# lutteropp/QuartetScores

Hardware: AMD Instinct MI355X
Metric: quartets counted/sec (higher is better)
Workload: dtype u32

## Files before the change

### quartetscores_amd/csrc/qs_count.hip

```cpp
#include "qs_common.hpp"
#include "qs_internal.hpp"
#include "qs_bitslice3.hpp"

#include <cstdio>
#include <cstdlib>
#include <type_traits>
#include <vector>

namespace qs {


constexpr int kPanelThreads = 256;
constexpr int kPanelPPT = 8;
constexpr int kPanelPB = kPanelThreads * kPanelPPT;

template <typename DT, bool PARTIAL>
__global__ __launch_bounds__(kPanelThreads) void build_panel_kernel(const uint32_t *__restrict__ leaf_off,
                                                                    const uint32_t *__restrict__ order, uint32_t slot0,
                                                                    const uint16_t *__restrict__ leaf_ids,
                                                                    const uint16_t *__restrict__ adj_depth,
                                                                    uint32_t n_trees, uint32_t n, uint32_t npairs,
                                                                    uint32_t levels, uint4 *__restrict__ P) {
    constexpr int TPC = 16 / (int)sizeof(DT);
    constexpr uint32_t FLAG = sizeof(DT) == 1 ? 0x20u : 0x2000u;
// ... 612 lines not shown
constexpr int c4_hi_words(int nwords) { return nwords <= 4 ? 0 : nwords == 5 ? 1 : nwords == 6 ? 2 : 4; }


template <int B> constexpr int bs4_waves() { return B <= 4 ? 5 : 4; }
template <int B, typename CT>
__global__ __launch_bounds__(kCountThreads) __attribute__((amdgpu_waves_per_eu(bs4_waves<B>(), bs4_waves<B>()))) void count_bitslice4_kernel(
    const uint4 *__restrict__ P, uint32_t npairs, uint32_t n_groups, uint32_t m_trees, uint32_t d_start, uint32_t d_hi,
    uint64_t rank_lo, uint32_t n_dblk, uint32_t n_slots, const uint32_t *__restrict__ dprefix, const uint32_t *__restrict__ cprefix,
    CT *__restrict__ table, uint32_t *__restrict__ overflow_flag, uint32_t overwrite, uint32_t xcd_remap, uint32_t *__restrict__ wire,
    const uint32_t *__restrict__ perm) {
    constexpr int NB = B + 1;
    constexpr int NWRAW = B < 4 ? 4 : B;
    constexpr int HR = c4_hi_words(NWRAW), HI = c4_hi_words(NB);
    __shared__ uint4 raw_lo[2][kC4Raw];
    __shared__ __align__(16) uint32_t raw_hi[2][HR ? kC4Raw * HR : 4];
    __shared__ uint4 img_lo[kWavesPerBlock][kWave];
    __shared__ __align__(16) uint32_t img_hi[kWavesPerBlock][HI ? kWave * HI : 4];

    const uint32_t lane = threadIdx.x & (kWave - 1);
    const uint32_t wave = __builtin_amdgcn_readfirstlane(threadIdx.x / kWave);
    uint32_t lb = blockIdx.x;
    if (xcd_remap & 1u) {
        const uint32_t nb = gridDim.x, q8 = nb / 8, r8 = nb % 8, xcd = lb % 8, y = lb / 8;
        lb = (xcd < r8 ? xcd * (q8 + 1) : r8 * (q8 + 1) + (xcd - r8) * q8) + y;
    }
    uint32_t tile = (uint32_t)__builtin_amdgcn_readfirstlane((int)perm[lb * kWavesPerBlock + wave]);
    const bool shadow = (tile & kShadowTile) != 0;
    tile &= ~kShadowTile;
    uint32_t dp_k, cp_c;
    const uint32_t k = wave_search_le(dprefix, 0, n_dblk, tile, lane, dp_k);
    const uint32_t local = tile - dp_k;
    const uint32_t d1 = d_hi - k * kDB;
    const uint32_t d0 = d1 > d_start + kDB ? d1 - kDB : d_start;
    const uint32_t c = wave_search_le(cprefix, 2, d1 - 1, local, lane, cp_c);
    const uint32_t tl = local - cp_c;
    uint32_t Bk = (uint32_t)(2.0f * sqrtf((float)tl + 1.0f));
    while ((Bk * Bk) / 4 > tl) --Bk;
    while (((Bk + 1) * (Bk + 1)) / 4 <= tl) ++Bk;
    const uint32_t jt = tl - (Bk * Bk) / 4;
    const uint32_t blk0 = 2 * jt, blk1 = 2 * jt + 1;
    const uint32_t ia = lane & (kTA - 1), ib = lane / kTA;
    const uint32_t a1 = blk0 * kTA + ia, a2 = blk1 * kTA + ia, b = Bk * kTB + ib;
    const bool v1 = !shadow && b < c, v2 = v1;
    const uint32_t pi1 = (uint32_t)binom2(b) + a1, pi2 = (uint32_t)binom2(b) + a2;
    const uint32_t jlo = c >= d0 ? c + 1 - d0 : 0u, jhi = d1 - d0;

    const uint32_t r_j = lane >> 3, r_col = lane & 7, dE = d0 + r_j;
    uint32_t shoff = kS3Inv;
    if (wave == 0) shoff = pi1 * 16u;
    else if (wave == 1) shoff = pi2 * 16u;
    else if (wave == 2) { const uint32_t bE = Bk * kTB + r_col; if (dE < d1 && bE < dE) shoff = ((uint32_t)binom2(dE) + bE) * 16u; }
    uint32_t pvoff = kS3Inv;
    if (lane < 16) { const uint32_t xa = (lane < 8 ? blk0 : blk1) * kTA + (lane & 7); if (xa < c) pvoff = ((uint32_t)binom2(c) + xa) * 16u; }
    else if (lane < 24) { const uint32_t dy = d0 + (lane - 16); if (dy < d1 && dy > c) pvoff = ((uint32_t)binom2(dy) + c) * 16u; }
    const uint32_t group_bytes = npairs * (uint32_t)(NWRAW * 4), hi_base = npairs * 16u;
    const uint32_t pv_slot = kC4Shared + wave * kC4Private;

    uint32_t x0[kDB], x1[kDB], y0[kDB], y1[kDB];
#pragma unroll
    for (int j = 0; j < kDB; ++j) x0[j] = x1[j] = y0[j] = y1[j] = 0;

    auto rsrc_of = [&](uint32_t g) {
        return __builtin_amdgcn_make_buffer_rsrc((void *)(reinterpret_cast<const char *>(P) + (size_t)g * group_bytes), 0, (int)group_bytes, 0x00020000);
    };
    auto put_raw = [&](int bufi, const Planes &sh, const Planes &pv) {
        if (wave < 3) c4_put<NWRAW>(raw_lo[bufi], raw_hi[bufi], wave * kWave + lane, sh);
        if (lane < kC4Private) c4_put<NWRAW>(raw_lo[bufi], raw_hi[bufi], pv_slot + lane, pv);
    };
    auto step = [&](uint32_t g_next, auto cur_tag, auto full_tag) {
        constexpr int CUR = decltype(cur_tag)::value;
        constexpr bool FULL = decltype(full_tag)::value;
        asm volatile("s_waitcnt lgkmcnt(0)\n\ts_barrier" ::: "memory");
        const Planes ab1 = c4_get<NWRAW>(raw_lo[CUR], raw_hi[CUR], lane);
        const Planes rowA1 = c4_get<NWRAW>(raw_lo[CUR], raw_hi[CUR], pv_slot + ia);
        const Planes ab2 = c4_get<NWRAW>(raw_lo[CUR], raw_hi[CUR], kWave + lane);
        const Planes rowA2 = c4_get<NWRAW>(raw_lo[CUR], raw_hi[CUR], pv_slot + 8 + ia);
        const Planes mbd = c4_get<NWRAW>(raw_lo[CUR], raw_hi[CUR], 2 * kWave + lane);
        const Planes mcd = c4_get<NWRAW>(raw_lo[CUR], raw_hi[CUR], pv_slot + 16 + r_j);
        const __amdgpu_buffer_rsrc_t r = rsrc_of(g_next);
        const Planes sh = buf_load_planes<NWRAW>(r, shoff, hi_base);
        const Planes pv = buf_load_planes<NWRAW>(r, pvoff, hi_base);
        c4_put<NB>(img_lo[wave], img_hi[wave], lane, sub_biased<B>(mbd, mcd));
        const Planes L1 = sub_biased<B>(ab1, rowA1);
        const Planes L2 = sub_biased<B>(ab2, rowA2);
#pragma unroll
        for (int j = 0; j < kDB; ++j) {
            if (FULL || ((uint32_t)j >= jlo && (uint32_t)j < jhi)) {
                const Planes Rb = c4_get<NB>(img_lo[wave], img_hi[wave], j * 8 + ib);
                uint32_t gt, lt, gt2, lt2;
                cmp_planes<NB>(L1, Rb, gt, lt);
                popc_acc(gt, x0[j]);
                popc_acc(lt, x1[j]);
                cmp_planes<NB>(L2, Rb, gt2, lt2);
                popc_acc(gt2, y0[j]);
                popc_acc(lt2, y1[j]);
            }
        }
        put_raw(CUR ^ 1, sh, pv);
    };
    auto run = [&](auto full_tag) {
        using Z_ = std::integral_constant<int, 0>; using O_ = std::integral_constant<int, 1>;
        {
            const __amdgpu_buffer_rsrc_t r = rsrc_of(0);
            put_raw(0, buf_load_planes<NWRAW>(r, shoff, hi_base), buf_load_planes<NWRAW>(r, pvoff, hi_base));
        }
        const uint32_t g_last = n_groups - 1;
        uint32_t g = 0;
        for (; g + 2 <= n_groups; g += 2) {
            step(g + 1, Z_{}, full_tag);
            step(min(g + 2, g_last), O_{}, full_tag);
        }
        if (g < n_groups) step(g_last, Z_{}, full_tag);
    };
    if (jlo == 0 && jhi == (uint32_t)kDB) run(std::true_type{}); else run(std::false_type{});

    uint64_t bd4 = binom4(d0), bd3 = binom3(d0), bd2 = binom2(d0);
    const uint64_t rcb = binom3(c) - rank_lo;
    if (wire) {
#pragma unroll
        for (int j = 0; j < kDB; ++j) {
            const uint32_t d = d0 + j;
            const uint64_t base = bd4 + rcb;
            bd4 += bd3; bd3 += bd2; bd2 += d;
            if (d < d1 && d > c && v1) {
                uint32_t w = x0[j] | (x1[j] << 16), w2 = y0[j] | (y1[j] << 16);
                if (!overwrite) { w += wire[base + pi1]; w2 += wire[base + pi2]; }
                wire[base + pi1] = w;
                wire[base + pi2] = w2;
            }
        }
        return;
    }
#pragma unroll
    for (int j = 0; j < kDB; ++j) {
        const uint32_t d = d0 + j;
        const uint64_t base = bd4 + rcb;
        bd4 += bd3; bd3 += bd2; bd2 += d;
        if (d < d1 && d > c && v1) {
            {
                const uint64_t idx = (base + pi1) * 3;
                uint32_t w0 = x0[j], w1 = x1[j], w2 = m_trees - x0[j] - x1[j];
                if (!overwrite) { const Tuple3<CT> t = load_tuple(table + idx); w0 += t.a; w1 += t.b; w2 += t.c; }
                if (sizeof(CT) == 2 && ((w0 | w1 | w2) > 0xFFFFu)) atomicOr(overflow_flag, 1u);
                store_tuple(table + idx, w0, w1, w2);
            }
            if (v2) {
                const uint64_t idx = (base + pi2) * 3;
                uint32_t w0 = y0[j], w1 = y1[j], w2 = m_trees - y0[j] - y1[j];
                if (!overwrite) { const Tuple3<CT> t = load_tuple(table + idx); w0 += t.a; w1 += t.b; w2 += t.c; }
                if (sizeof(CT) == 2 && ((w0 | w1 | w2) > 0xFFFFu)) atomicOr(overflow_flag, 1u);
                store_tuple(table + idx, w0, w1, w2);
            }
        }
    }
}


hipError_t launch_count_bitslice3(hipStream_t s, const CountGeometry &g_in, const void *panel, int depth_bits, int mode,
                                  uint32_t n_groups, uint32_t m_trees, void *table, int count_bits, uint32_t *overflow_flag,
                                  bool overwrite, uint32_t *wire) {
    if (g_in.total_tiles == 0 || n_groups == 0) return hipSuccess;
    const uint32_t npairs = (uint32_t)binom2(g_in.n);
    CountGeometry g = g_in;
    if (mode == MODE_BINARY_FULL && g.perm_coop && g.n_coop && depth_bits <= 7) {
        dim3 grid4(g.n_coop / kWavesPerBlock), block4(kCountThreads);
#define QS_BS4(BB, CT)                                                                                              \
    hipLaunchKernelGGL((count_bitslice4_kernel<BB, CT>), grid4, block4, 0, s, (const uint4 *)panel, npairs, n_groups, m_trees, \
                       g.d_lo, g.d_hi, g.rank_lo, g.n_dblk, g.n_coop, g.dprefix, g.cprefix, (CT *)table, overflow_flag,    \
                       overwrite ? 1u : 0u, 1u, wire, g.perm_coop)
#define QS_BS4_B(CT)                                                                                                \
    do {                                                                                                            \
        if (depth_bits <= 4) QS_BS4(4, CT);                                                                         \
        else if (depth_bits == 5) QS_BS4(5, CT);                                                                    \
        else if (depth_bits == 6) QS_BS4(6, CT);                                                                    \
        else QS_BS4(7, CT);                                                                                         \
    } while (0)
        if (count_bits == 32) QS_BS4_B(uint32_t); else QS_BS4_B(uint16_t);
#undef QS_BS4_B
#undef QS_BS4
        hipError_t e4 = hipGetLastError();
        if (e4 != hipSuccess) return e4;
        g.perm = g.perm_rest; g.total_tiles = g.n_rest;
        if (g.total_tiles == 0) return hipSuccess;
    }
    dim3 grid((g.total_tiles + kWavesPerBlock - 1) / kWavesPerBlock), block(kCountThreads);
#define QS_BS3(BB, MM, CT)                                                                                          \
    hipLaunchKernelGGL((count_bitslice3_kernel<BB, MM, CT>), grid, block, 0, s, (const uint4 *)panel, npairs, n_groups, \
                       m_trees, g.d_lo, g.d_hi, g.rank_lo, g.n_dblk, g.total_tiles, g.dprefix, g.cprefix,           \
                       (CT *)table, overflow_flag, overwrite ? 1u : 0u, g.n >= 200 ? (((kSyncModes >> (MM)) & 1u) ? 3u : 1u) : 0u , wire, g.perm)
#define QS_BS3_B(MM, CT)                                                                                            \
    do {                                                                                                            \
        switch (depth_bits <= 4 ? 4 : depth_bits) {                                                                 \
            case 4: QS_BS3(4, MM, CT); break;                                                                       \
            case 5: QS_BS3(5, MM, CT); break;                                                                       \
            case 6: QS_BS3(6, MM, CT); break;                                                                       \
            case 7: QS_BS3(7, MM, CT); break;                                                                       \
            case 8: QS_BS3(8, MM, CT); break;                                                                       \
            case 9: QS_BS3(9, MM, CT); break;                                                                       \
            default: QS_BS3(10, MM, CT); break;                                                                     \
        }                                                                                                           \
    } while (0)
#define QS_BS3_BP(CT) QS_BS3_B(MODE_PARTIAL, CT)
    if (depth_bits > kMaxDepthBits) return hipErrorInvalidValue;
    if (count_bits == 32) {
        if (mode == MODE_BINARY_FULL) QS_BS3_B(MODE_BINARY_FULL, uint32_t);
        else if (mode == MODE_GENERAL_FULL) QS_BS3_B(MODE_GENERAL_FULL, uint32_t);
        else if (mode == MODE_BINARY_PARTIAL) QS_BS3_B(MODE_BINARY_PARTIAL, uint32_t);
        else QS_BS3_BP(uint32_t);
    } else {
        if (mode == MODE_BINARY_FULL) QS_BS3_B(MODE_BINARY_FULL, uint16_t);
        else if (mode == MODE_GENERAL_FULL) QS_BS3_B(MODE_GENERAL_FULL, uint16_t);
        else if (mode == MODE_BINARY_PARTIAL) QS_BS3_B(MODE_BINARY_PARTIAL, uint16_t);
        else QS_BS3_BP(uint16_t);
    }
#undef QS_BS3_BP
#undef QS_BS3_B
#undef QS_BS3
    return hipGetLastError();
}



template <typename CT> __device__ __forceinline__ void table_atomic_inc(CT *table, uint64_t cell, uint32_t *overflow_flag);
template <> __device__ __forceinline__ void table_atomic_inc<uint32_t>(uint32_t *table, uint64_t cell, uint32_t *) {
    atomicAdd(&table[cell], 1u);
}
template <> __device__ __forceinline__ void table_atomic_inc<uint16_t>(uint16_t *table, uint64_t cell, uint32_t *overflow_flag) {
    uint32_t *w = reinterpret_cast<uint32_t *>(table) + (cell >> 1);
    const uint32_t old = atomicAdd(w, (cell & 1) ? 0x10000u : 1u);
    if (((cell & 1) ? old >> 16 : old & 0xFFFFu) == 0xFFFFu) atomicOr(overflow_flag, 1u);
}

constexpr int kScatterMaxLeaves = 4096;

template <typename CT>
__global__ __launch_bounds__(kWave) void count_scatter_kernel(const uint32_t *__restrict__ leaf_off,
                                                              const uint16_t *__restrict__ leaf_ids,
                                                              const uint32_t *__restrict__ node_tree,
                                                              const uint32_t *__restrict__ rng_off,
                                                              const uint16_t *__restrict__ ranges, uint32_t d_lo,
                                                              uint32_t d_hi, uint64_t rank_lo, CT *__restrict__ table,
                                                              uint32_t *__restrict__ overflow_flag) {
    __shared__ uint16_t ids[kScatterMaxLeaves];
    const uint32_t v = blockIdx.x, lane = threadIdx.x;
    const uint32_t t = node_tree[v];
    const uint32_t base = leaf_off[t], L = leaf_off[t + 1] - base;
    for (uint32_t i = lane; i < L; i += kWave) ids[i] = leaf_ids[base + i];
    __syncthreads();
    const uint32_t k0 = rng_off[v], k = rng_off[v + 1] - k0;
    for (uint32_t i1 = 0; i1 < k; ++i1)
        for (uint32_t i2 = i1 + 1; i2 < k; ++i2)
            for (uint32_t i3 = i2 + 1; i3 < k; ++i3) {
                const uint32_t li[3] = {i1, i2, i3};
                for (int o = 0; o < 3; ++o) {
                    const uint32_t lp = li[o], lq = li[(o + 1) % 3], lr = li[(o + 2) % 3];
                    const uint32_t ps = ranges[2 * (k0 + lp)], pe = ranges[2 * (k0 + lp) + 1];
                    const uint32_t qs_ = ranges[2 * (k0 + lq)], qe = ranges[2 * (k0 + lq) + 1];
                    const uint32_t rs = ranges[2 * (k0 + lr)], re = ranges[2 * (k0 + lr) + 1];
                    const uint32_t np = (pe + L - ps) % L, nq = (qe + L - qs_) % L, nr = (re + L - rs) % L;
                    for (uint32_t x = 0; x < np; ++x) {
                        const uint32_t a = ids[(ps + x) % L];
                        for (uint32_t y = x + 1; y < np; ++y) {
                            const uint32_t a2 = ids[(ps + y) % L];
                            const uint32_t amin = min(a, a2);
                            for (uint32_t z = 0; z < nq; ++z) {
                                const uint32_t bq = ids[(qs_ + z) % L];
                                if (bq < amin) continue;
                                for (uint32_t w = lane; w < nr; w += kWave) {
                                    const uint32_t cr = ids[(rs + w) % L];
                                    if (cr < amin) continue;
                                    uint32_t s0 = min(a, a2), s1 = max(a, a2), s2 = min(bq, cr), s3 = max(bq, cr);
                                    uint32_t lo = min(s1, s2), hi = max(s1, s2);
                                    uint32_t m1 = lo, m2 = min(hi, s3), m3 = max(hi, s3);
                                    if (m3 < d_lo || m3 >= d_hi) continue;
                                    const int slot = slot_of_pairing(a, a2, bq, cr);
                                    const uint64_t cell = (rank4(s0, m1, m2, m3) - rank_lo) * 3 + (uint64_t)slot;
                                    table_atomic_inc<CT>(table, cell, overflow_flag);
                                }
                            }
                        }
                    }
                }
            }
}

hipError_t launch_count_scatter(hipStream_t s, const DeviceBatch &b, uint32_t n, uint32_t d_lo, uint32_t d_hi,
                                uint64_t rank_lo, void *table, int count_bits, uint32_t *overflow_flag) {
    (void)n;
    if (b.n_nodes == 0) return hipSuccess;
    dim3 grid(b.n_nodes), block(kWave);
    if (count_bits == 32)
        hipLaunchKernelGGL(count_scatter_kernel<uint32_t>, grid, block, 0, s, b.leaf_off, b.leaf_ids, b.node_tree, b.rng_off,
                           b.ranges, d_lo, d_hi, rank_lo, (uint32_t *)table, overflow_flag);
    else
        hipLaunchKernelGGL(count_scatter_kernel<uint16_t>, grid, block, 0, s, b.leaf_off, b.leaf_ids, b.node_tree, b.rng_off,
                           b.ranges, d_lo, d_hi, rank_lo, (uint16_t *)table, overflow_flag);
    return hipGetLastError();
}

constexpr int kFixMaxRun = 128;
constexpr int kFixThreads = 256;
enum FixRule { FIX_BINARY = 0, FIX_GENERAL = 1, FIX_WIRE = 2 };

template <typename CT> __device__ __forceinline__ void table_atomic_dec(CT *table, uint64_t cell, uint32_t *overflow_flag);
template <> __device__ __forceinline__ void table_atomic_dec<uint32_t>(uint32_t *table, uint64_t cell, uint32_t *) { atomicSub(&table[cell], 1u); }
template <> __device__ __forceinline__ void table_atomic_dec<uint16_t>(uint16_t *table, uint64_t cell, uint32_t *overflow_flag) {
    uint32_t *w = reinterpret_cast<uint32_t *>(table) + (cell >> 1);
    const uint32_t old = atomicSub(w, (cell & 1) ? 0x10000u : 1u);
    if (((cell & 1) ? old >> 16 : old & 0xFFFFu) == 0u) atomicOr(overflow_flag, 1u);
}

template <typename CT, int RULE>
__global__ __launch_bounds__(kFixThreads) void clamp_fix_kernel(const FixUnit *__restrict__ units, const uint32_t *__restrict__ leaf_off,
                                                                const uint16_t *__restrict__ leaf_ids, const uint16_t *__restrict__ adj_depth,
                                                                uint32_t d_lo, uint32_t d_hi, uint64_t rank_lo, CT *__restrict__ table,
                                                                uint32_t *__restrict__ wire, uint32_t *__restrict__ overflow_flag) {
    __shared__ uint16_t ids[kScatterMaxLeaves];
    __shared__ uint16_t rm[kFixMaxRun][kFixMaxRun];
    const FixUnit u = units[blockIdx.x];
    const uint32_t tid = threadIdx.x;
    const uint32_t base = leaf_off[u.tree], L = leaf_off[u.tree + 1] - base;
    const uint32_t i0 = u.run & 0xFFFFu, s = u.run >> 16;
    for (uint32_t i = tid; i < L; i += kFixThreads) ids[i] = leaf_ids[base + i];
    for (uint32_t a = tid; a + 1 < s; a += kFixThreads) {
        uint32_t m = 0xFFFFu;
        for (uint32_t b = a + 1; b < s; ++b) { m = min(m, (uint32_t)adj_depth[base + i0 + b - 1]); rm[a][b] = (uint16_t)m; }
    }
    __syncthreads();
    uint32_t k = 2, rest = u.t_lo;
    while ((uint32_t)binom3(k + 1) <= rest) ++k;
    rest -= (uint32_t)binom3(k);
    uint32_t j = 1;
    while ((uint32_t)binom2(j + 1) <= rest) ++j;
    uint32_t i = rest - (uint32_t)binom2(j);
    const uint32_t n_out = L - s;
    for (uint32_t t = u.t_lo; t < u.t_hi; ++t) {
        const uint32_t mij = rm[i][j], mjk = rm[j][k];
        const uint32_t x1 = ids[i0 + i], x2 = ids[i0 + j], x3 = ids[i0 + k];
        const uint32_t n_in = s - 1 - k;
        const uint32_t q0 = mij != mjk ? 0u : n_out;
        for (uint32_t q = q0 + tid; q < n_out + n_in; q += kFixThreads) {
            uint32_t pa, pb, oa, ob;
            if (q < n_out) {
                const uint32_t x = ids[q < i0 ? q : q + s];
                if (mij > mjk) { pa = x1; pb = x2; oa = x3; ob = x; } else { pa = x2; pb = x3; oa = x1; ob = x; }
            } else {
                const uint32_t l = k + 1 + (q - n_out), x4 = ids[i0 + l];
                const uint32_t mkl = rm[k][l], mx = max(mij, mkl);
                if (mjk < mx) { pa = x1; pb = x2; oa = x3; ob = x4; }
                else if (mjk > mx) { pa = x1; pb = x4; oa = x2; ob = x3; }
                else continue;
            }
            const uint32_t lo1 = min(pa, pb), hi1 = max(pa, pb), lo2 = min(oa, ob), hi2 = max(oa, ob);
            const uint32_t s0 = min(lo1, lo2), s3 = max(hi1, hi2), m1 = max(lo1, lo2), m2 = min(hi1, hi2);
            if (s3 < d_lo || s3 >= d_hi) continue;
            const uint32_t s1 = min(m1, m2), s2 = max(m1, m2);
            const int slot = slot_of_pairing(pa, pb, oa, ob);
            const uint64_t tup = rank4(s0, s1, s2, s3) - rank_lo;
            if (RULE == FIX_WIRE) { if (slot < 2) atomicAdd(&wire[tup], slot ? 0x10000u : 1u); }
            else if (RULE == FIX_GENERAL) table_atomic_inc<CT>(table, tup * 3 + (uint64_t)slot, overflow_flag);
            else if (slot != 2) { table_atomic_inc<CT>(table, tup * 3 + (uint64_t)slot, overflow_flag); table_atomic_dec<CT>(table, tup * 3 + 2, overflow_flag); }
        }
        if (++i == j) { i = 0; if (++j == k) { j = 1; ++k; } }
    }
}

hipError_t launch_clamp_fix(hipStream_t s, const DeviceBatch &b, const FixUnit *units, uint32_t n_units, uint32_t d_lo, uint32_t d_hi,
                            uint64_t rank_lo, void *table, int count_bits, int mode, uint32_t *wire, uint32_t *overflow_flag) {
    if (n_units == 0) return hipSuccess;
    dim3 grid(n_units), block(kFixThreads);
    const bool gen = mode == MODE_GENERAL_FULL || mode == MODE_PARTIAL;
#define QS_FIX(CT, RULE) hipLaunchKernelGGL((clamp_fix_kernel<CT, RULE>), grid, block, 0, s, units, b.leaf_off, b.leaf_ids, b.adj_depth, d_lo, d_hi, rank_lo, (CT *)table, wire, overflow_flag)
    if (wire) QS_FIX(uint32_t, FIX_WIRE);
    else if (count_bits == 32) { if (gen) QS_FIX(uint32_t, FIX_GENERAL); else QS_FIX(uint32_t, FIX_BINARY); }
    else { if (gen) QS_FIX(uint16_t, FIX_GENERAL); else QS_FIX(uint16_t, FIX_BINARY); }
#undef QS_FIX
    return hipGetLastError();
}

__global__ __launch_bounds__(256) void pack16_kernel(const uint32_t *__restrict__ src, uint32_t *__restrict__ dst,
                                                     uint64_t n_words, uint64_t n_cells, uint32_t *__restrict__ overflow_flag) {
    const uint64_t i = (uint64_t)blockIdx.x * blockDim.x + threadIdx.x;
    if (i >= n_words) return;
    const uint32_t lo = src[2 * i];
    const uint32_t hi = (2 * i + 1 < n_cells) ? src[2 * i + 1] : 0u;
    if ((lo | hi) > 0xFFFFu) atomicOr(overflow_flag, 1u);
    dst[i] = (lo & 0xFFFFu) | (hi << 16);
}

__global__ __launch_bounds__(256) void pack16x2_kernel(const uint32_t *__restrict__ src, uint32_t *__restrict__ dst,
                                                       uint64_t n_tuples, uint32_t trees, uint32_t *__restrict__ overflow_flag,
                                                       uint32_t *__restrict__ shape_flag) {
    const uint64_t i = (uint64_t)blockIdx.x * blockDim.x + threadIdx.x;
    if (i >= n_tuples) return;
    const uint32_t n0 = src[3 * i], n1 = src[3 * i + 1], n2 = src[3 * i + 2];
    if ((n0 | n1) > 0xFFFFu) atomicOr(overflow_flag, 1u);
    if (n0 + n1 + n2 != trees) atomicOr(shape_flag, 1u);
    dst[i] = (n0 & 0xFFFFu) | (n1 << 16);
}
__global__ __launch_bounds__(256) void unpack16x2_kernel(const uint32_t *__restrict__ src, uint16_t *__restrict__ dst,
                                                         uint64_t n_tuples, uint32_t trees, uint32_t *__restrict__ shape_flag) {
    const uint64_t i = (uint64_t)blockIdx.x * blockDim.x + threadIdx.x;
    if (i >= n_tuples) return;
    const uint32_t w = src[i], n0 = w & 0xFFFFu, n1 = w >> 16;
    if (n0 + n1 > trees) atomicOr(shape_flag, 1u);
    dst[3 * i] = (uint16_t)n0; dst[3 * i + 1] = (uint16_t)n1; dst[3 * i + 2] = (uint16_t)(trees - n0 - n1);
}
__global__ __launch_bounds__(256) void pack32x2_kernel(const uint32_t *__restrict__ src, uint2 *__restrict__ dst, uint64_t n_tuples,
                                                       uint32_t trees, uint32_t *__restrict__ shape_flag) {
    const uint64_t i = (uint64_t)blockIdx.x * blockDim.x + threadIdx.x;
    if (i >= n_tuples) return;
    const uint32_t n0 = src[3 * i], n1 = src[3 * i + 1], n2 = src[3 * i + 2];
    if (n0 + n1 + n2 != trees) atomicOr(shape_flag, 1u);
    dst[i] = make_uint2(n0, n1);
}
__global__ __launch_bounds__(256) void unpack32x2_kernel(const uint2 *__restrict__ src, uint32_t *__restrict__ dst, uint64_t n_tuples,
                                                         uint32_t trees, uint32_t *__restrict__ shape_flag) {
    const uint64_t i = (uint64_t)blockIdx.x * blockDim.x + threadIdx.x;
    if (i >= n_tuples) return;
    const uint2 w = src[i];
    if ((uint64_t)w.x + w.y > trees) atomicOr(shape_flag, 1u);
    dst[3 * i] = w.x; dst[3 * i + 1] = w.y; dst[3 * i + 2] = trees - w.x - w.y;
}
hipError_t launch_pack32x2(hipStream_t s, const void *table_u32, void *dst, uint64_t n_tuples, uint32_t trees, uint32_t *shape_flag) {
    if (n_tuples == 0) return hipSuccess;
    dim3 block(256), grid((unsigned)((n_tuples + 255) / 256));
    hipLaunchKernelGGL(pack32x2_kernel, grid, block, 0, s, (const uint32_t *)table_u32, (uint2 *)dst, n_tuples, trees, shape_flag);
    return hipGetLastError();
}
hipError_t launch_unpack32x2(hipStream_t s, const void *src, void *dst_u32, uint64_t n_tuples, uint32_t trees, uint32_t *shape_flag) {
    if (n_tuples == 0) return hipSuccess;
    dim3 block(256), grid((unsigned)((n_tuples + 255) / 256));
    hipLaunchKernelGGL(unpack32x2_kernel, grid, block, 0, s, (const uint2 *)src, (uint32_t *)dst_u32, n_tuples, trees, shape_flag);
    return hipGetLastError();
}
hipError_t launch_pack16x2(hipStream_t s, const void *table_u32, void *dst, uint64_t n_tuples, uint32_t trees,
                           uint32_t *overflow_flag, uint32_t *shape_flag) {
    if (n_tuples == 0) return hipSuccess;
    dim3 block(256), grid((unsigned)((n_tuples + 255) / 256));
    hipLaunchKernelGGL(pack16x2_kernel, grid, block, 0, s, (const uint32_t *)table_u32, (uint32_t *)dst, n_tuples, trees, overflow_flag, shape_flag);
    return hipGetLastError();
}
hipError_t launch_unpack16x2(hipStream_t s, const void *src, void *dst_u16, uint64_t n_tuples, uint32_t trees, uint32_t *shape_flag) {
    if (n_tuples == 0) return hipSuccess;
    dim3 block(256), grid((unsigned)((n_tuples + 255) / 256));
    hipLaunchKernelGGL(unpack16x2_kernel, grid, block, 0, s, (const uint32_t *)src, (uint16_t *)dst_u16, n_tuples, trees, shape_flag);
    return hipGetLastError();
}

constexpr int kSumMaxSrc = 15;
struct SumSources { const uint32_t *p[kSumMaxSrc]; };
__global__ __launch_bounds__(256) void sum_words_kernel(uint32_t *__restrict__ dst, SumSources src, uint32_t n_src, uint64_t n_words) {
    const uint64_t n4 = n_words / 4, stride = (uint64_t)gridDim.x * blockDim.x;
    for (uint64_t i = (uint64_t)blockIdx.x * blockDim.x + threadIdx.x; i < n4; i += stride) {
        qs_u32x4 acc = reinterpret_cast<const qs_u32x4 *>(dst)[i];
        for (uint32_t k = 0; k < n_src; ++k) acc += __builtin_nontemporal_load(reinterpret_cast<const qs_u32x4 *>(src.p[k]) + i);
        reinterpret_cast<qs_u32x4 *>(dst)[i] = acc;
    }
    const uint64_t t = 4 * n4 + (uint64_t)blockIdx.x * blockDim.x + threadIdx.x;
    if (t < n_words) {
        uint32_t acc = dst[t];
        for (uint32_t k = 0; k < n_src; ++k) acc += src.p[k][t];
        dst[t] = acc;
    }
}
hipError_t launch_sum_words(hipStream_t s, void *dst, const void *const *src, uint32_t n_src, uint64_t n_words, int n_cu) {
    if (n_words == 0 || n_src == 0) return hipSuccess;
    if (n_src > (uint32_t)kSumMaxSrc) return hipErrorInvalidValue;
    SumSources ss;
    for (uint32_t k = 0; k < (uint32_t)kSumMaxSrc; ++k) ss.p[k] = k < n_src ? (const uint32_t *)src[k] : nullptr;
    const uint64_t want = (n_words / 4 + 255) / 256;
    dim3 block(256), grid((unsigned)std::max<uint64_t>(1, std::min<uint64_t>(want, (uint64_t)std::max(n_cu, 1) * 16)));
    hipLaunchKernelGGL(sum_words_kernel, grid, block, 0, s, (uint32_t *)dst, ss, n_src, n_words);
    return hipGetLastError();
}

hipError_t launch_pack16(hipStream_t s, const void *table_u32, void *dst, uint64_t n_cells, uint32_t *overflow_flag) {
    const uint64_t n_words = (n_cells + 1) / 2;
    if (n_words == 0) return hipSuccess;
    dim3 block(256), grid((unsigned)((n_words + 255) / 256));
    hipLaunchKernelGGL(pack16_kernel, grid, block, 0, s, (const uint32_t *)table_u32, (uint32_t *)dst, n_words, n_cells, overflow_flag);
    return hipGetLastError();
}


template <typename CT>
__global__ void lookup_kernel(uint32_t d_lo, uint32_t d_hi, uint64_t rank_lo, const CT *__restrict__ table, uint64_t nq,
                              const uint16_t *__restrict__ abcd, uint64_t *__restrict__ out) {
    const uint64_t i = (uint64_t)blockIdx.x * blockDim.x + threadIdx.x;
    if (i >= nq) return;
    const uint32_t a = abcd[4 * i], b = abcd[4 * i + 1], c = abcd[4 * i + 2], d = abcd[4 * i + 3];
    uint32_t lo1 = min(a, b), hi1 = max(a, b), lo2 = min(c, d), hi2 = max(c, d);
    uint32_t s0 = min(lo1, lo2), s3 = max(hi1, hi2);
    uint32_t m1 = max(lo1, lo2), m2 = min(hi1, hi2);
    uint32_t s1 = min(m1, m2), s2 = max(m1, m2);
    uint64_t o0 = 0, o1 = 0, o2 = 0;
    if (s3 >= d_lo && s3 < d_hi && s0 != s1 && s1 != s2 && s2 != s3) {
        const uint64_t cell = (rank4(s0, s1, s2, s3) - rank_lo) * 3;
        o0 = table[cell + slot_of_pairing(a, b, c, d)];
        o1 = table[cell + slot_of_pairing(a, c, b, d)];
        o2 = table[cell + slot_of_pairing(a, d, b, c)];
    }
    out[3 * i] = o0; out[3 * i + 1] = o1; out[3 * i + 2] = o2;
}

hipError_t launch_lookup(hipStream_t s, uint32_t n, uint32_t d_lo, uint32_t d_hi, uint64_t rank_lo, const void *table,
                         int count_bits, uint64_t nq, const uint16_t *abcd_dev, uint64_t *out_dev) {
    (void)n;
    if (nq == 0) return hipSuccess;
    dim3 block(256), grid((unsigned)((nq + 255) / 256));
    if (count_bits == 32)
        hipLaunchKernelGGL(lookup_kernel<uint32_t>, grid, block, 0, s, d_lo, d_hi, rank_lo, (const uint32_t *)table, nq,
                           abcd_dev, out_dev);
    else
        hipLaunchKernelGGL(lookup_kernel<uint16_t>, grid, block, 0, s, d_lo, d_hi, rank_lo, (const uint16_t *)table, nq,
                           abcd_dev, out_dev);
    return hipGetLastError();
}

}
```

Baseline: 95380 billion.

## Shrink clamp-fix LDS footprint, sort outside leaves, split inc/dec across threads

The clamp-fix kernel now stores the range-min matrix in triangular form, which roughly halves its LDS use and should let more blocks fit per CU. Leaves outside the run are gathered through a shared bitmap into sorted order, which may improve locality of the table atomics. In binary mode, each increment/decrement pair is split across two threads through a unified atomic step helper, so twice as many threads issue atomics. This adds extra syncthreads and a serial prefix-popcount pass, and it assumes leaf ids within a tree are unique.

```diff
diff --git a/quartetscores_amd/csrc/qs_count.hip b/quartetscores_amd/csrc/qs_count.hip
--- a/quartetscores_amd/csrc/qs_count.hip
+++ b/quartetscores_amd/csrc/qs_count.hip
@@ -938,12 +938,15 @@
 constexpr int kFixThreads = 256;
 enum FixRule { FIX_BINARY = 0, FIX_GENERAL = 1, FIX_WIRE = 2 };
 
-template <typename CT> __device__ __forceinline__ void table_atomic_dec(CT *table, uint64_t cell, uint32_t *overflow_flag);
-template <> __device__ __forceinline__ void table_atomic_dec<uint32_t>(uint32_t *table, uint64_t cell, uint32_t *) { atomicSub(&table[cell], 1u); }
-template <> __device__ __forceinline__ void table_atomic_dec<uint16_t>(uint16_t *table, uint64_t cell, uint32_t *overflow_flag) {
+template <typename CT> __device__ __forceinline__ void table_atomic_step(CT *table, uint64_t cell, uint32_t dec, uint32_t *overflow_flag);
+template <> __device__ __forceinline__ void table_atomic_step<uint32_t>(uint32_t *table, uint64_t cell, uint32_t dec, uint32_t *) {
+    atomicAdd(&table[cell], dec ? 0xFFFFFFFFu : 1u);
+}
+template <> __device__ __forceinline__ void table_atomic_step<uint16_t>(uint16_t *table, uint64_t cell, uint32_t dec, uint32_t *overflow_flag) {
     uint32_t *w = reinterpret_cast<uint32_t *>(table) + (cell >> 1);
-    const uint32_t old = atomicSub(w, (cell & 1) ? 0x10000u : 1u);
-    if (((cell & 1) ? old >> 16 : old & 0xFFFFu) == 0u) atomicOr(overflow_flag, 1u);
+    const uint32_t one = (cell & 1) ? 0x10000u : 1u;
+    const uint32_t old = atomicAdd(w, dec ? 0u - one : one);
+    if (((cell & 1) ? old >> 16 : old & 0xFFFFu) == (dec ? 0u : 0xFFFFu)) atomicOr(overflow_flag, 1u);
 }
 
 template <typename CT, int RULE>
@@ -951,16 +954,32 @@
                                                                 const uint16_t *__restrict__ leaf_ids, const uint16_t *__restrict__ adj_depth,
                                                                 uint32_t d_lo, uint32_t d_hi, uint64_t rank_lo, CT *__restrict__ table,
                                                                 uint32_t *__restrict__ wire, uint32_t *__restrict__ overflow_flag) {
-    __shared__ uint16_t ids[kScatterMaxLeaves];
-    __shared__ uint16_t rm[kFixMaxRun][kFixMaxRun];
+    constexpr uint32_t kWords = kScatterMaxLeaves / 32;
+    __shared__ uint16_t oid[kScatterMaxLeaves];
+    __shared__ uint16_t rid[kFixMaxRun];
+    __shared__ uint32_t present[kWords + 1];
+    __shared__ uint16_t rm[kFixMaxRun * (kFixMaxRun - 1) / 2];
     const FixUnit u = units[blockIdx.x];
     const uint32_t tid = threadIdx.x;
     const uint32_t base = leaf_off[u.tree], L = leaf_off[u.tree + 1] - base;
     const uint32_t i0 = u.run & 0xFFFFu, s = u.run >> 16;
-    for (uint32_t i = tid; i < L; i += kFixThreads) ids[i] = leaf_ids[base + i];
+    if (tid < kWords) present[tid] = 0u;
+    __syncthreads();
+    for (uint32_t i = tid; i < L; i += kFixThreads) {
+        const uint32_t id = leaf_ids[base + i];
+        if (i - i0 < s) rid[i - i0] = (uint16_t)id;
+        else atomicOr(&present[(id >> 5) & (kWords - 1)], 1u << (id & 31));
+    }
     for (uint32_t a = tid; a + 1 < s; a += kFixThreads) {
         uint32_t m = 0xFFFFu;
-        for (uint32_t b = a + 1; b < s; ++b) { m = min(m, (uint32_t)adj_depth[base + i0 + b - 1]); rm[a][b] = (uint16_t)m; }
+        for (uint32_t b = a + 1; b < s; ++b) { m = min(m, (uint32_t)adj_depth[base + i0 + b - 1]); rm[b * (b - 1) / 2 + a] = (uint16_t)m; }
+    }
+    __syncthreads();
+    if (tid < kWords) {
+        uint32_t o = 0;
+        for (uint32_t w = 0; w < tid; ++w) o += __popc(present[w]);
+        for (uint32_t bits = present[tid]; bits; bits &= bits - 1) oid[o++] = (uint16_t)(tid * 32 + __ffs(bits) - 1);
+        if (tid == kWords - 1) present[kWords] = o;
     }
     __syncthreads();
     uint32_t k = 2, rest = u.t_lo;
@@ -969,20 +988,22 @@
     uint32_t j = 1;
     while ((uint32_t)binom2(j + 1) <= rest) ++j;
     uint32_t i = rest - (uint32_t)binom2(j);
-    const uint32_t n_out = L - s;
+    const uint32_t n_out = present[kWords];
+    constexpr uint32_t kOps = RULE == FIX_BINARY ? 2u : 1u, kSweep = kFixThreads / kOps;
+    const uint32_t qt = tid / kOps, op = tid % kOps;
     for (uint32_t t = u.t_lo; t < u.t_hi; ++t) {
-        const uint32_t mij = rm[i][j], mjk = rm[j][k];
-        const uint32_t x1 = ids[i0 + i], x2 = ids[i0 + j], x3 = ids[i0 + k];
+        const uint32_t mij = rm[j * (j - 1) / 2 + i], mjk = rm[k * (k - 1) / 2 + j];
+        const uint32_t x1 = rid[i], x2 = rid[j], x3 = rid[k];
         const uint32_t n_in = s - 1 - k;
         const uint32_t q0 = mij != mjk ? 0u : n_out;
-        for (uint32_t q = q0 + tid; q < n_out + n_in; q += kFixThreads) {
+        for (uint32_t q = q0 + qt; q < n_out + n_in; q += kSweep) {
             uint32_t pa, pb, oa, ob;
             if (q < n_out) {
-                const uint32_t x = ids[q < i0 ? q : q + s];
+                const uint32_t x = oid[q];
                 if (mij > mjk) { pa = x1; pb = x2; oa = x3; ob = x; } else { pa = x2; pb = x3; oa = x1; ob = x; }
             } else {
-                const uint32_t l = k + 1 + (q - n_out), x4 = ids[i0 + l];
-                const uint32_t mkl = rm[k][l], mx = max(mij, mkl);
+                const uint32_t l = k + 1 + (q - n_out), x4 = rid[l];
+                const uint32_t mkl = rm[l * (l - 1) / 2 + k], mx = max(mij, mkl);
                 if (mjk < mx) { pa = x1; pb = x2; oa = x3; ob = x4; }
                 else if (mjk > mx) { pa = x1; pb = x4; oa = x2; ob = x3; }
                 else continue;
@@ -995,7 +1016,7 @@
             const uint64_t tup = rank4(s0, s1, s2, s3) - rank_lo;
             if (RULE == FIX_WIRE) { if (slot < 2) atomicAdd(&wire[tup], slot ? 0x10000u : 1u); }
             else if (RULE == FIX_GENERAL) table_atomic_inc<CT>(table, tup * 3 + (uint64_t)slot, overflow_flag);
-            else if (slot != 2) { table_atomic_inc<CT>(table, tup * 3 + (uint64_t)slot, overflow_flag); table_atomic_dec<CT>(table, tup * 3 + 2, overflow_flag); }
+            else if (slot != 2) table_atomic_step<CT>(table, tup * 3 + (op ? 2u : (uint64_t)slot), op, overflow_flag);
         }
         if (++i == j) { i = 0; if (++j == k) { j = 1; ++k; } }
     }
```

Measured after the change: 96180 billion (median of 6 runs). No clear change (+0.8%).
